# couchbase/blance

Measured on AMD Instinct MI355X. Metric: partition-state assignments/sec at 1M partitions x 4,096 nodes, higher is better.
Workload: dtype f64

## Files before the change

### __graft_entry__.py

```python
import os
import subprocess
import sys

ROOT = os.path.dirname(os.path.abspath(__file__))
if ROOT not in sys.path:
    sys.path.insert(0, ROOT)

CSRC = os.path.join(ROOT, "blance_amd", "csrc")
HIP_TUS = ["blance_hip.hip", "tu_seq.hip", "tu_tree.hip", "tu_queue.hip", "tu_chain.hip", "tu_batch.hip"]
HIP_LIB = os.path.join(ROOT, "blance_amd", "lib", "libblance_hip.so")
HIP_OBJ = os.path.join(ROOT, "blance_amd", "lib", "obj")
HIPCC_FLAGS = ["--offload-arch=gfx950", "-O3", "-std=c++17", "-ffp-contract=off", "-fPIC"]


def _stale(target, deps):
    return (not os.path.exists(target)) or any(os.path.getmtime(d) > os.path.getmtime(target) for d in deps)


def depfile_entries(path):
    try:
        with open(path) as f:
            text = f.read()
    except OSError:
        return None
# ... 159 lines not shown
    if not force and stamp is not None and os.path.exists(lib) and _read(lib + ".stamp") == stamp:
        return lib
    os.makedirs(os.path.dirname(lib), exist_ok=True)
    hipcc = os.environ.get("HIPCC", "/opt/rocm/bin/hipcc")
    for old in (lib + ".d", lib + ".deps", lib + ".stamp"):
        if os.path.exists(old):
            os.remove(old)
    r = subprocess.run([hipcc] + HIPCC_FLAGS + ["-shared", "-MD", "-MF", lib + ".d", "-o", lib, src],
                       stderr=subprocess.PIPE, text=True)
    if r.returncode != 0:
        err = "\n".join(l for l in (r.stderr or "").splitlines() if "error" in l.lower())
        raise RuntimeError("hipcc failed on %s\n%s" % (src, err[-4000:]))
    deps = depfile_entries(lib + ".d") or []
    rels = sorted(set(os.path.relpath(os.path.realpath(d), os.path.realpath(ROOT)) for d in deps if not d.startswith(("/opt/", "/usr/"))))
    with open(lib + ".deps", "w") as f:
        f.write("\n".join(rels) + "\n")
    with open(lib + ".stamp", "w") as f:
        f.write(_small_stamp(lib))
    return lib


def build_stay_rank_cases(force=False):
    return _build_small_cases(RANKS_SRC, RANKS_LIB, force)


PERIOD_SRC = os.path.join(CASES_DIR, "period_cases.hip")
PERIOD_LIB = os.path.join(CASES_DIR, "_build", "libblance_period_cases.so")


def build_period_cases(force=False):
    return _build_small_cases(PERIOD_SRC, PERIOD_LIB, force)


def build_host():
    host = os.path.join(ROOT, "blance_amd", "csrc", "host")
    srcs = [os.path.join(host, "blance_host_cli.cpp"), os.path.join(host, "blance_api.cpp"), os.path.join(host, "call_arena.cpp")]
    out = os.path.join(ROOT, "blance_amd", "lib", "blance_host_cli")
    if _stale(out, srcs + [os.path.join(host, "blance_api.hpp"), os.path.join(host, "call_arena.hpp"),
                           os.path.join(ROOT, "include", "blance_hip.h")]):
        subprocess.check_call(["g++", "-std=c++17", "-O2", "-pthread", "-DBLANCE_CALL_ARENA", "-o", out] + srcs + ["-ldl"])
    build_wire()
    build_move_index()
    return out


def build_move_index():
    host = os.path.join(ROOT, "blance_amd", "csrc", "host")
    src, hdr = os.path.join(host, "move_index_sim.cpp"), os.path.join(host, "move_index.hpp")
    out = os.path.join(ROOT, "blance_amd", "lib", "move_index_sim")
    if _stale(out, [src, hdr]):
        subprocess.check_call(["g++", "-std=c++17", "-O2", "-o", out, src])
    return out


def build_wire():
    src = os.path.join(ROOT, "blance_amd", "csrc", "host", "blance_wire.cpp")
    out = os.path.join(ROOT, "blance_amd", "lib", "libblance_wire.so")
    if _stale(out, [src, os.path.join(ROOT, "include", "blance_wire.h"),
                    os.path.join(ROOT, "blance_amd", "csrc", "host", "json_escape.hpp")]):
        subprocess.check_call(["g++", "-std=c++17", "-O2", "-fPIC", "-shared", "-I", os.path.join(ROOT, "include"),
                               "-o", out, src])
    return out


def build():
    with_cases = os.path.exists(CASES_SRC) and all(os.path.exists(os.path.join(CASES_DIR, inc)) for inc in CASES_INCS)
    cases = start_kernel_cases() if with_cases else None
    try:
        build_hip()
    except BaseException:
        if cases is not None:
            cases.kill()
        raise
    if with_cases:
        build_kernel_cases(cases)
    if os.path.exists(RANKS_SRC):
        build_stay_rank_cases()
    if os.path.exists(PERIOD_SRC):
        build_period_cases()
    build_host()
    from oracle import loader, naive_loader
    loader.build()
    naive_loader.build()
    from blance_amd import hip
    lib = hip.load_library()
    assert lib.blance_abi_version() == 6
    import blance_amd


def smoke():
    from blance_amd import hip, synth
    from oracle import loader
    fp = synth.config_flat(3, P=2048, N=256)
    pl = hip.Planner(device_id=0)
    got = pl.plan(fp)
    want = loader.plan(fp)
    assert got.digest() == want.digest(), "HIP result differs from the oracle"
    assert got.iterations == want.iterations
    fp2 = synth.config_flat(2, P=4096, N=64)
    assert pl.plan(fp2).digest() == loader.plan(fp2).digest()
    fp3 = synth.config5_initial(3000, 128)
    r3 = pl.plan(fp3)
    assert r3.digest() == loader.plan(fp3).digest(), "config-5-shaped plan differs from the oracle"
    fp4 = synth.config5_rebalance(fp3, r3, 3000, 128)
    assert pl.plan(fp4).digest() == loader.plan(fp4).digest(), "config-5-shaped rebalance differs from the oracle"
    pl.close()
    print("smoke ok: iterations=%d device_ms=%.3f" % (got.iterations, got.struct.device_ms))


if __name__ == "__main__":
    build()
    if len(sys.argv) > 1 and sys.argv[1] == "smoke":
# ... 2 lines not shown
```

### blance_amd/csrc/blance_hip.hip

```cpp
#include "dev_prelude.h"

#include <algorithm>
#include <atomic>
#include <chrono>
#include <map>
#include <mutex>
#include <new>
#include <thread>
#include <type_traits>
#include <string>
#include <vector>

#include "k_sweep.h"
#include "k_flat.h"
#include "k_period.h"
#include "k_plan_moves.h"
#include "k_plan_wire.h"
#include "host/json_escape.hpp"
#ifdef BLANCE_SIMT_EMU
#include "tu_seq.hip"
#include "tu_tree.hip"
#include "tu_queue.hip"
#include "tu_chain.hip"
#include "tu_batch.hip"
#endif


using namespace blance;

static thread_local std::string g_last_error;

static int fail(int code, const char* fmt, const char* a = "", long b = 0) {
    char buf[512];
    snprintf(buf, sizeof buf, fmt, a, b);
    g_last_error = buf;
    return code;
}

#define HIPTRY(expr)                                                                  \
    do {                                                                              \
        hipError_t e_ = (expr);                                                       \
        if (e_ != hipSuccess)                                                         \
            return fail(BLANCE_ERR_DEVICE, "%s failed: line %ld", hipGetErrorString(e_), __LINE__); \
    } while (0)

struct DevBuf {
    void* p = nullptr;
    size_t cap = 0;
// ... 168 lines not shown
};

constexpr int kChainHandoffMin = 8192;

enum PassKind { kPassKernel = 0, kPassFlatBulk = 1, kPassBlank = 2, kPassStayTop = 3 };

struct blance_ctx : CtxHandles {
    int device = 0;
    int engine = BLANCE_ENGINE_AUTO;
    int force_threads = 0;
    std::mutex mu;
    bool uploaded = false;
    bool planned = false;
    blance_comm comm{0, 1, nullptr, nullptr, nullptr};
    void* rccl_comm = nullptr;
    DevBuf scan_sums;
    DevBuf scan_part;
    DevBuf topkey, top_counts, top_off, top_order;
    DevBuf side_sums;
    bool side_pending = false;
    int top_group_state = -1;
    int64_t top_group_epoch = -1, group_epoch = 0;
    std::vector<int64_t> last_stays;
    int chain_handoff = kChainHandoffMin;
    DevBuf handoff;
    bool no_stay_top = false;
    bool force_stay_top = false;
    bool periodic = true;
    int periodic_cut = 0;
    bool period_known = true;
    uint32_t assign_kinds = 0;
    bool cycle_order_stands = false;
    bool leaves_distinct = false;
    DevBuf cnt_base, xbuf, gath;
    std::vector<int32_t> h_reg_off;
    int chain_group_state = -1;
    bool chain_group_static = false;
    bool tops_moved = true;
    uint32_t top_gate = 0;
    bool flags_clean = false;
    bool rowcount_clean = false;
    bool top_prio_strict = false;
    bool uniform_first = false, uniform_all = false;
    bool trace = false;
    int dump_sweep = -1;
    DevBuf dl_off, dl_nodes;
    HostStage stage;
    void* rb_buf = nullptr;
    size_t rb_used = 0;
    struct RbItem { void* dst; size_t off, bytes; };
    std::vector<RbItem> rb_items;
    DevBuf vres, vseen;
    DevBuf mv[11];
    bool wire_names = false;
    int wire_stage = kWireStageDefault;
    DevBuf wire[10];
    int64_t comm_calls = 0, comm_bytes = 0;
    size_t comm_events_used = 0;
    double comm_ms = 0.0;
    int64_t n_syncs = 0;
    bool assign_empty = false, counts_start_zero = false;
    int chain_waves = 0;
    int speculate = 1;
    bool fused_tail = true;

    blance_problem h{};
    std::vector<int32_t> state_priority, state_constraints, rule_off;
    int L = 1, np_later = 0, n_alive = 0, any_removed = 0;
    int chain_min_parts = 2048;
    int any_node_weight = 0;
    bool no_fast_keys = false;
    bool no_seq_spec = false;
    bool no_tree = false;
    bool tree_dense = false;
    bool tree_always = false;
    bool tree_long = false;
    bool no_planes = false;
    bool no_queue = false;
    bool queue_general = false;
    bool queue_no_asm = false;
    bool queue_force_dense = false;
    bool queue_exact_rebuild = false;
    bool queue_bits_self = false;
    bool shard_one_rank = false;
    DevBuf ntn_bits;
    bool bits_stale = false;
    bool pass_ntn_ready = false;
    int64_t queue_launches = 0, queue_stops = 0, queue_moved = 0, queue_exact = 0, queue_rebuilds = 0, queue_dense = 0;
    struct RuleRegions {
        bool ok = false;
        int n_regions = 0, max_size = 0;
        DevBuf node_region, reg_lo, reg_hi, leaf_cls, cls_size;
        DevBuf wg_region, wg_chunk;
        int n_stay_wgs = 0, n_leaves = 0;
        int cls_run = 0;
    };
    std::vector<RuleRegions> rule_regions;
    DevBuf leaf_node, regid, chain_order, bucket_counts, reg_off, cnt_save, crec;
    DevBuf chain_inv;
    DevBuf period, cnt_p1;
    DevBuf fl_iota, fl_zero, fl_one, fl_reglo, fl_reghi;
    DevBuf n_ev, chain_oi, ev_key, ev_oi, ev_leaf, ev_w, ev_perm, ev_off, ev_counts;
    bool flat_chain_ok = false;
    DevBuf f_tot, f_g, f_top_g, f_top_n, f_row_count, f_m, f_moff, f_keys_a, f_keys_b, f_vals_a, f_vals_b, f_hist, f_comp;
    int64_t out_capacity = 0;
    DevBuf batch_in, batch_sc, batch_out;

    DevBuf node_removed, node_added, node_weight, node_has_weight, alive, zeros_nx, node_leaf_pos;
    DevBuf alive_ids, alive_rank;
    DevBuf part_order, part_weight, part_has_weight, part_in_prev, part_never_equal;
    DevBuf a_off, a_nodes, a_kind, p_off, p_nodes, p_kind;
    DevBuf load_state, load_node, load_weight, load_first;
    DevBuf rule_inc, rule_exc, vparent, vlo, vhi, anchors;
    DevBuf state_stick, state_has_stick;
    DevBuf live, live_len, live_kind, prv, prv_len, prv_kind, in_prev, never_equal;
    DevBuf cnt, ntn, cat, order, chunk_counts, rec, out, warn_part, warn_state, scalars;
    DevBuf cnt_next;
    bool tail_counted = false;
    PlanStats stats;
    ~blance_ctx();
    std::vector<PassKind> pass_kind;
};

static void comm_release(blance_ctx* c);
template <class F>
static int guarded(F f) {
    try {
        return f();
// ... 150 lines not shown
    if (!out) return fail(BLANCE_ERR_BAD_ARG, "null out");
    *out = nullptr;
    int n_dev = 0;
    if (hipGetDeviceCount(&n_dev) != hipSuccess || n_dev <= 0)
        return fail(BLANCE_ERR_NO_DEVICE, "no HIP device visible");
    int dev = opt ? opt->device_id : 0;
    if (dev < 0 || dev >= n_dev) return fail(BLANCE_ERR_BAD_ARG, "device_id out of range");
    HIPTRY(hipSetDevice(dev));
    blance_ctx* c = new blance_ctx();
    c->device = dev;
    c->engine = opt ? opt->engine : BLANCE_ENGINE_AUTO;
    c->force_threads = opt ? opt->reserved[0] : 0;
    if (opt && opt->reserved[1] > 0) c->chain_min_parts = opt->reserved[1];
    c->no_seq_spec = opt && (opt->reserved[2] & 1);
    c->no_tree = opt && (opt->reserved[2] & 2);
    c->tree_dense = opt && (opt->reserved[2] & 4);
    c->tree_always = opt && (opt->reserved[2] & 8);
    c->tree_long = opt && (opt->reserved[2] & 16);
    c->no_planes = opt && (opt->reserved[2] & 32);
    c->no_queue = opt && (opt->reserved[2] & 512);
    c->queue_general = opt && (opt->reserved[2] & 1024);
    c->queue_force_dense = opt && (opt->reserved[2] & 2048);
    c->queue_no_asm = opt && (opt->reserved[2] & 4096);
    c->queue_exact_rebuild = opt && (opt->reserved[2] & 8192);
    c->shard_one_rank = opt && (opt->reserved[2] & 16384);
    c->queue_bits_self = opt && (opt->reserved[2] & 32768);
    c->no_stay_top = opt && (opt->reserved[2] & 64);
    c->force_stay_top = opt && (opt->reserved[2] & 128);
    c->periodic = !(opt && (opt->reserved[2] & 256));
    if (const char* pe = getenv("BLANCE_PERIODIC")) c->periodic = atoi(pe) != 0;
    if (const char* pc = getenv("BLANCE_PERIODIC_CUT")) c->periodic_cut = atoi(pc);
    c->period_known = !(opt && (opt->reserved[2] & 65536));
    if (const char* pk = getenv("BLANCE_PERIOD_KNOWN")) c->period_known = atoi(pk) != 0;
    c->trace = getenv("BLANCE_TRACE") != nullptr;
    if (const char* cw = getenv("BLANCE_CHAIN_WAVES")) c->chain_waves = atoi(cw);
    if (const char* ho = getenv("BLANCE_CHAIN_HANDOFF")) c->chain_handoff = atoi(ho) > 0 ? atoi(ho) : 0;
    if (const char* sp = getenv("BLANCE_SPECULATE")) c->speculate = !strcmp(sp, "fail") ? 2 : atoi(sp) != 0;
    if (const char* ft = getenv("BLANCE_FUSED_TAIL")) c->fused_tail = atoi(ft) != 0;
    if (const char* ds = getenv("BLANCE_DUMP_SWEEP")) c->dump_sweep = atoi(ds);
    if (const char* ws = getenv("BLANCE_WIRE_STAGE")) {
        const int v = atoi(ws);
        c->wire_stage = v < kWireStageMin ? kWireStageMin : v > kWireStageMax ? kWireStageMax : v;
    }
    if (hipStreamCreate(&c->stream) != hipSuccess || hipEventCreate(&c->ev0) != hipSuccess ||
        hipEventCreate(&c->ev1) != hipSuccess ||
        hipEventCreate(&c->side_go) != hipSuccess || hipEventCreate(&c->side_done) != hipSuccess) {
        delete c;
        return fail(BLANCE_ERR_DEVICE, "stream/event creation failed");
    }
    *out = c;
    g_live_contexts++;
    return BLANCE_OK;
}

blance_ctx::~blance_ctx() {
    (void)hipSetDevice(device);
    if (stream) (void)hipStreamSynchronize(stream);
    if (side) (void)hipStreamSynchronize(side);
    comm_release(this);
    if (rb_buf) pin_free(rb_buf);
}

extern "C" void blance_ctx_destroy(blance_ctx* c) {
    if (!c) return;
    delete c;
    if (--g_live_contexts == 0) pin_trim();
// ... 360 lines not shown
                    if (sz != cls_run || sz < 1 || sz > 64 || (sz & (sz - 1)) || (cl[i].first - rlo[g]) % sz) cls_run = 0;
                    for (int lp = cl[i].first; lp < cl[i].second && cls_run > 0; lp++) if (leaf_node[lp] < 0) cls_run = 0;
                }
                for (size_t i = 0; i < cl.size() && ok; i++) cls_size[rlo[g] + i] = cl[i].second - cl[i].first;
                for (int lp = rlo[g]; lp < rhi[g] && ok; lp++) {
                    int a = leaf_node[lp];
                    if (a < 0) continue;
                    size_t j = std::upper_bound(cl.begin(), cl.end(), std::make_pair(lp, INT_MAX)) - cl.begin();
                    if (j > 0 && lp < cl[j - 1].second) {
                        if (t[a].blo != cl[j - 1].first || t[a].bhi != cl[j - 1].second) ok = false;
                        leaf_cls[lp] = (int)j - 1;
                    }
                }
            }
            rr.ok = ok;
            rr.n_regions = ok ? (int)rlo.size() : 0;
            rr.max_size = max_size;
            rr.n_leaves = n_leaves;
            rr.cls_run = ok && cls_run > 0 ? cls_run : 0;
            std::vector<int32_t> wg_region, wg_chunk;
            if (ok)
                for (size_t g = 0; g < rlo.size(); g++)
                    for (int ch = 0; ch * 64 < rhi[g] - rlo[g]; ch++) { wg_region.push_back((int32_t)g); wg_chunk.push_back(ch); }
            rr.n_stay_wgs = (int)wg_region.size();
            if (ok) {
                if (put(up, rr.wg_region, wg_region.data(), wg_region.size())) return BLANCE_ERR_DEVICE;
                if (put(up, rr.wg_chunk, wg_chunk.data(), wg_chunk.size())) return BLANCE_ERR_DEVICE;
                if (put(up, rr.node_region, node_region.data(), node_region.size())) return BLANCE_ERR_DEVICE;
                if (put(up, rr.reg_lo, rlo.data(), rlo.size())) return BLANCE_ERR_DEVICE;
                if (put(up, rr.reg_hi, rhi.data(), rhi.size())) return BLANCE_ERR_DEVICE;
                if (put(up, rr.leaf_cls, leaf_cls.data(), leaf_cls.size())) return BLANCE_ERR_DEVICE;
                if (put(up, rr.cls_size, cls_size.data(), cls_size.size())) return BLANCE_ERR_DEVICE;
            }
            if ((st = up.flush())) return st;
        }
        if ((st = up.flush())) return st;
    }
    const int RW = kRecHead + M * (1 + L);
    int kmax = 1;
    for (int m = 0; m < M; m++) if (pb->state_constraints[m] > kmax) kmax = pb->state_constraints[m];
    RESERVE(live, sizeof(int32_t) * (size_t)(PM * L + 1));
    RESERVE(live_len, sizeof(int32_t) * (size_t)(PM + 1));
    RESERVE(live_kind, (size_t)PM + 1);
    RESERVE(prv, sizeof(int32_t) * (size_t)(PM * L + 1));
    RESERVE(prv_len, sizeof(int32_t) * (size_t)(PM + 1));
    RESERVE(prv_kind, (size_t)PM + 1);
    RESERVE(in_prev, (size_t)P + 1);
    RESERVE(never_equal, (size_t)P + 1);
    RESERVE(cnt, sizeof(int32_t) * (size_t)(M + 1) * (NX + 1));
    RESERVE(cnt_next, sizeof(int32_t) * (size_t)(M + 1) * (NX + 1));
    RESERVE(ntn, sizeof(int32_t) * (size_t)(NX + 1) * (N > 0 ? N : 1));
    RESERVE(cat, (size_t)P + 1);
    RESERVE(order, sizeof(int32_t) * ((size_t)P + 1));
    RESERVE(chunk_counts, sizeof(int32_t) * 3 * (size_t)(cdiv(P, kPartChunk) + 1));
    RESERVE(rec, sizeof(int32_t) * ((size_t)P * RW + 64));
    RESERVE(out, sizeof(int32_t) * ((size_t)P * (1 + kmax) + 1));
    RESERVE(warn_part, sizeof(int32_t) * (size_t)(PM + 1));
    RESERVE(warn_state, sizeof(int32_t) * (size_t)(PM + 1));
    RESERVE(scalars, sizeof(int32_t) * kScalWords);
    RESERVE(ntn_bits, sizeof(uint32_t) * (queue_bits_words(NX) + 4));
    {
        int maxB = 1;
        for (auto& rr : c->rule_regions) if (rr.ok && rr.n_regions > maxB) maxB = rr.n_regions;
        RESERVE(regid, sizeof(int32_t) * ((size_t)P + 1));
        RESERVE(chain_order, sizeof(int32_t) * ((size_t)P + 1));
        RESERVE(chain_inv, sizeof(int32_t) * ((size_t)P + 1));
// ... 730 lines not shown
    d.live = d.prv; d.live_len = d.prv_len; d.live_kind = d.prv_kind;
    return d;
}

static DevProblem dev_problem(blance_ctx* c) {
    const blance_problem& h = c->h;
    DevProblem d;
    d.N = h.n_nodes; d.NX = h.n_nodes_ext; d.M = h.n_states; d.L = c->L; d.P = h.n_parts;
    d.weights_nil = h.partition_weights_nil;
    d.node_removed = c->zeros_nx.as<uint8_t>();
    d.node_added = c->zeros_nx.as<uint8_t>();
    d.part_weight = c->part_weight.as<int32_t>();
    d.part_has_weight = c->part_has_weight.as<uint8_t>();
    d.live = c->live.as<int32_t>(); d.live_len = c->live_len.as<int32_t>(); d.live_kind = c->live_kind.as<uint8_t>();
    d.prv = c->prv.as<int32_t>(); d.prv_len = c->prv_len.as<int32_t>(); d.prv_kind = c->prv_kind.as<uint8_t>();
    d.in_prev = c->in_prev.as<uint8_t>(); d.never_equal = c->never_equal.as<uint8_t>();
    return d;
}

constexpr int kXHead = 16, kXPoison = kChainFlags;
struct SweepTail {
    bool set = false, scatter = false;
    int m = 0, OW = 0;
    const int32_t* order = nullptr;
    const int32_t* inv = nullptr;
    Gate gate = kNoGate;
};
struct ChainPassArgs {
    int m, k, NP, higher_mask, r0, it;
    const int32_t* order;
    bool same_tops;
    SweepTail* tail;
    bool known_cycle = false;
};

static void comm_poison(blance_ctx* c) {
    const blance_problem& h = c->h;
    const size_t n = kXHead + (size_t)(h.n_states + 1) * h.n_nodes_ext;
    if (c->xbuf.reserve(sizeof(int32_t) * (n + 1))) return;
    if (hipMemsetAsync(c->xbuf.p, 0, sizeof(int32_t) * n, c->stream) != hipSuccess) return;
    const int32_t one = 1;
    if (hipMemcpyAsync(c->xbuf.as<int32_t>() + kXPoison, &one, sizeof one, hipMemcpyHostToDevice, c->stream) != hipSuccess) return;
    if (stream_sync(c) != hipSuccess) return;
    (void)comm_allreduce(c, c->xbuf.as<int32_t>(), (int64_t)n);
    (void)stream_sync(c);
}

struct Progress {
    int64_t steps = 0, batched = 0;
    int n_pass = 0;
    int passes_this_sweep = 0;
};
struct PlanRun {
    DevProblem d;
    int64_t launches = 0;
    Progress at;
    int32_t hs[kScalReadback] = {0};
    int m_last = -1;
    bool fuse = false;
    bool top_spec_plan = true;
    bool handoff_plan = true;
    int iterations = 0, converged = 0;
};

enum class Pending { kNone, kStayTop, kBlank, kChain };
struct ChainRun {
    bool allow_spec = true, defer = false, no_stay = false, no_lean = false, skip = false;
    bool no_handoff = false;
    bool handoff = false;
    bool redo_handoff = false;
    bool redo = false;
    Pending pending = Pending::kNone;
    bool spec = false;
    Gate gate = kNoGate;
    bool done = false;
    bool a_done = false;
};

struct ChainPass {
    blance_ctx* const c;
    PlanRun& pr;
    const ChainPassArgs& a;
    ChainRun& run;
    const blance_problem& h;
    const DevProblem& d;
    blance_ctx::RuleRegions& rr;
    const int m, OW, P, B, nbc, G, rank;
    const bool sharded;
    const size_t cnt_words;
    const hipStream_t sm;
    int32_t* const flags;
    Gate top_gate = kNoGate;
    bool regroup = false, spec = false, defer = false, gather_out = false;
    int32_t cfl[kChainFlags] = {0};
    int32_t n_events = 0;
    bool stay_fits = false, try_stay = false, group_stands = false, group_ahead = false;
    bool handoff = false;
    ChainParams cq;

    ChainPass(blance_ctx* c_, PlanRun& pr_, const ChainPassArgs& a_, ChainRun& run_)
        : c(c_), pr(pr_), a(a_), run(run_), h(c_->h), d(pr_.d), rr(c_->rule_regions[a_.r0]), m(a_.m), OW(1 + a_.k), P(c_->h.n_parts), B(rr.n_regions),
          nbc(cdiv(c_->h.n_parts, kPartChunk)), G(c_->comm.n_ranks), rank(c_->comm.rank), sharded(pass_sharded(c_, rr.n_regions)),
          cnt_words((size_t)(c_->h.n_states + 1) * c_->h.n_nodes_ext), sm(c_->stream),
          flags(c_->scalars.as<int32_t>() + kScalFlags) {}

    int slice_lo(int r) const { return (int)((int64_t)B * r / G); }
    Gate gate_on(uint32_t words) const {
        return Gate{flags, words | (1u << kFlagForced) | (spec ? (1u << kFlagOrphans) | (1u << kFlagEvents) : 0u) | c->top_gate};
    }
    bool refuted(const int32_t* f) const { return spec && (f[kFlagOrphans] || f[kFlagEvents] || c->speculate == 2); }
    void uncount_orphans() {
        BLANCE_LAUNCH_NOSYNC(k_chain_orphans, cdiv(P, 256), 256, 0, sm, d, m, h.top_state, a.order,
                             rr.node_region.as<int32_t>(), c->cnt.as<int32_t>());
    }
    int restore_counters() {
        HIPTRY(hipMemcpyAsync(c->cnt.p, c->cnt_save.p, sizeof(int32_t) * cnt_words, hipMemcpyDeviceToDevice, sm));
        return 0;
    }
    int open_timing() { HIPTRY(hipEventRecord(c->pass_events[2 * pr.at.n_pass], sm)); return 0; }
    int close_timing(PassKind kind) {
        HIPTRY(hipEventRecord(c->pass_events[2 * pr.at.n_pass + 1], sm));
        c->pass_kind.resize(pr.at.n_pass + 1);
        c->pass_kind[pr.at.n_pass] = kind;
        pr.at.n_pass++;
        return 0;
    }

    int classify_and_group();
    int events();
    int gather_records();
    int group_by_top(hipStream_t st, DevBuf& sums);
    void fill_chain_params();
    int start_counters();
    void fill_stay_params(StayParams& sq);
    int stay_attempt(bool* stayed);
    int stay_behind_handoff();
    int trace_handoff();
    int longest_chain() const {
        int mx = 0;
        if (c->h_reg_off.size() == (size_t)B + 1)
            for (int r = 0; r < B; r++) mx = std::max(mx, (int)(c->h_reg_off[r + 1] - c->h_reg_off[r]));
        return mx;
    }
    int blank_walk(bool* lean);
    int periodic_walk(bool* walked);
    int collective_a(int32_t* fl);
    int collective_b();
    int commit();
    int run_once();
};

int ChainPass::classify_and_group() {
    if (!c->flags_clean) HIPTRY(hipMemsetAsync(flags, 0, sizeof(int32_t) * kChainFlags, sm));
    c->flags_clean = false;
    top_gate = Gate{flags, c->top_gate};
    regroup = !(a.same_tops && c->chain_group_state == m && c->chain_group_static && a.order == c->part_order.as<int32_t>() &&
                c->h_reg_off.size() == (size_t)B + 1);
    spec = run.allow_spec && !regroup && !sharded && c->speculate > 0;
    if (!spec) {
        const LaunchShape cs = shape_chain_classify(P);
        BLANCE_LAUNCH_NOSYNC(k_chain_classify, cs.grid, cs.block, cs.lds, sm, d, m, h.top_state,
                             a.order, rr.node_region.as<int32_t>(), c->regid.as<int32_t>(),
                             c->n_ev.as<int32_t>(), flags, top_gate);
    } else {
        if (c->trace) fprintf(stderr, "[blance] chain pass state %d: no k_chain_classify, k_gather_chain raises its flag words\n", m);
    }
    if (regroup) {
        const int ge = group_by_key(c, sm, c->scan_sums, P, c->regid.as<int32_t>(), a.order, B, c->bucket_counts.as<int32_t>(),
                                    c->reg_off.as<int32_t>(), c->chain_order.as<int32_t>(), c->chain_oi.as<int32_t>());
        if (ge) return ge;
        BLANCE_LAUNCH_NOSYNC(k_invert, cdiv(P, 256), 256, 0, sm, P, c->chain_order.as<int32_t>(), c->chain_inv.as<int32_t>());
        pr.launches++;
        c->chain_group_state = m;
        c->group_epoch++;
        c->chain_group_static = a.order == c->part_order.as<int32_t>();
    } else if (c->trace) fprintf(stderr, "[blance] chain pass state %d: the grouping by region of the last sweep stands\n", m);
    defer = run.defer && !sharded && c->speculate > 0;
    if (c->top_gate && (regroup || !spec || !defer))
        return fail(BLANCE_ERR_DEVICE, "a chain pass behind the top-state pass's verdict would read back");
    run.spec = spec;
    run.pending = Pending::kNone;
    run.redo = false;
    if (!spec) {
        HIPTRY(read_back(c, cfl, flags, sizeof cfl));
        if (regroup) {
            c->h_reg_off.resize((size_t)B + 1);
            HIPTRY(read_back(c, c->h_reg_off.data(), c->reg_off.p, sizeof(int32_t) * ((size_t)B + 1)));
        }
        HIPTRY(stream_sync(c));
    }
    return 0;
}

int ChainPass::events() {
    if (!cfl[kFlagNotLocal] && cfl[kFlagEvents]) {
        SCANTRY(P + 1, c->n_ev.as<int32_t>());
        HIPTRY(read_back(c, &n_events, c->n_ev.as<int32_t>() + P, sizeof n_events));
        HIPTRY(stream_sync(c));
    }
    if (c->trace)
        fprintf(stderr, spec ? "[blance] chain pass state %d: classification assumed clean (checked with the pass's flags)\n" :
                               "[blance] chain pass state %d: %d events, not-local %d, orphans %d\n", m, n_events, cfl[kFlagNotLocal], cfl[kFlagOrphans]);
    {
        FillCopyJob fj;
        fj.zero(c->ev_off.p, (int64_t)B + 1);
        fj.zero(flags + kFlagStayMoved, 1);
        fj.zero(flags + kFlagHandedOff, 1);
        fj.copy(c->cnt_save.p, c->cnt.p, (int64_t)cnt_words);
        if (run_fill_copy(c, fj)) return BLANCE_ERR_DEVICE;
    }
    if (!cfl[kFlagNotLocal] && n_events > 0) {
        BLANCE_LAUNCH_NOSYNC(k_chain_ev_fill, cdiv(P, 256), 256, 0, sm, d, m, h.top_state, a.order,
                             rr.node_region.as<int32_t>(), rr.reg_lo.as<int32_t>(), c->node_leaf_pos.as<int32_t>(),
                             c->regid.as<int32_t>(), c->n_ev.as<int32_t>(), c->ev_key.as<int32_t>(),
                             c->ev_oi.as<int32_t>(), c->ev_leaf.as<int32_t>(), c->ev_w.as<int32_t>());
        const int ge = group_by_key(c, sm, c->scan_sums, n_events, c->ev_key.as<int32_t>(), nullptr, B, c->ev_counts.as<int32_t>(),
                                    c->ev_off.as<int32_t>(), c->ev_perm.as<int32_t>(), nullptr);
        if (ge) return ge;
        pr.launches += 5;
    }
    return 0;
}

int ChainPass::group_by_top(hipStream_t st, DevBuf& sums) {
    const int ge = group_by_key(c, st, sums, P, c->topkey.as<int32_t>(), nullptr, rr.n_leaves, c->top_counts.as<int32_t>(),
                                c->top_off.as<int32_t>(), c->top_order.as<int32_t>(), nullptr);
    if (ge) return ge;
    c->top_group_state = m;
    c->top_group_epoch = c->group_epoch;
    pr.launches += 5;
    return 0;
}

int ChainPass::gather_records() {
    const bool fits_but_np = !sharded && !c->no_stay_top && !cfl[kFlagNotLocal] && !cfl[kFlagOrphans] && !cfl[kFlagEvents] &&
                             rr.max_size <= kStayMaxLeaves && rr.n_stay_wgs > 0;
    stay_fits = fits_but_np && a.NP > 0;
    try_stay = stay_fits && !run.no_stay && (c->force_stay_top || c->last_stays[m] * 100 >= (int64_t)P * 99);
    const bool handoff_plan_ok = c->chain_handoff > 0 && pr.handoff_plan && c->speculate > 0 && !run.no_handoff && run.allow_spec &&
                                 longest_chain() - 64 * 4 >= c->chain_handoff;
    handoff = stay_fits && !try_stay && handoff_plan_ok && chain_rows_in_lds(cq, rr.max_size);
    const bool handoff_next = fits_but_np && a.NP == 0 && c->np_later > 0 && handoff_plan_ok && a.it + 1 < h.max_iterations;
    group_stands = c->top_group_state == m && c->top_group_epoch == c->group_epoch;
    const bool for_next = stay_fits && !try_stay && c->speculate > 0 && a.it + 1 < h.max_iterations;
    group_ahead = (for_next || handoff || handoff_next) && !group_stands && (c->side || g_live_contexts.load() <= 2);
    if (group_ahead && !c->side && hipStreamCreate(&c->side) != hipSuccess) { c->side = nullptr; group_ahead = false; (void)hipGetLastError(); }
    const bool group_here = (handoff || handoff_next) && !group_stands && !group_ahead;
    if (try_stay || group_ahead || handoff || group_here) {
        RESERVE(topkey, sizeof(int32_t) * ((size_t)P + 1));
        RESERVE(top_order, sizeof(int32_t) * ((size_t)P + 1));
        RESERVE(top_off, sizeof(int32_t) * ((size_t)rr.n_leaves + 2));
        RESERVE(top_counts, sizeof(int32_t) * ((size_t)rr.n_leaves * nbc + 1));
        if (c->side_pending) {
            HIPTRY(hipStreamWaitEvent(sm, c->side_done, 0));
            c->side_pending = false;
        }
    }
    const bool group_now = (try_stay && !group_stands) || group_ahead || group_here;
    const LaunchShape gs = shape_gather_chain(P);
    BLANCE_LAUNCH(k_gather_chain, gs.grid, gs.block, gs.lds, sm, d, m, h.top_state, a.higher_mask,
                         c->chain_order.as<int32_t>(), c->chain_oi.as<int32_t>(), c->state_stick.as<int32_t>(),
                         c->state_has_stick.as<uint8_t>(), c->node_leaf_pos.as<int32_t>(),
                         rr.node_region.as<int32_t>(), rr.reg_lo.as<int32_t>(), rr.leaf_cls.as<int32_t>(),
                         rr.cls_size.as<int32_t>(), 0, spec ? 1 : 0,
                         c->crec.as<int32_t>(), flags, group_now ? c->topkey.as<int32_t>() : (int32_t*)nullptr, top_gate);
    if (group_ahead) {
        HIPTRY(hipEventRecord(c->side_go, sm));
        HIPTRY(hipStreamWaitEvent(c->side, c->side_go, 0));
        const int ge = group_by_top(c->side, c->side_sums);
        if (ge) return ge;
        HIPTRY(hipEventRecord(c->side_done, c->side));
        c->side_pending = true;
        if (c->trace) fprintf(stderr, "[blance] chain pass state %d: the steps grouped by top priority node for the next sweep, on the second stream\n", m);
    } else if (group_here) {
        const int ge = group_by_top(sm, c->scan_sums);
        if (ge) return ge;
        if (c->trace) fprintf(stderr, "[blance] chain pass state %d: the steps grouped by top priority node for the hand-off\n", m);
    }
    return 0;
}

void ChainPass::fill_chain_params() {
    fill_pass_common(c, cq, m, a.k, a.NP);
    fill_region_tables(c, rr, cq);
    cq.L = c->L;
    cq.n_regions = B;
    cq.waves = c->chain_waves ? c->chain_waves : (a.it == 0 ? 4 : 0);
    cq.cls_run = rr.cls_run;
    cq.region_base = sharded ? slice_lo(rank) : 0;
    cq.n_launch = sharded ? slice_lo(rank + 1) - cq.region_base : B;
    cq.reg_off = c->reg_off.as<int32_t>();
    cq.ntn = c->ntn.as<int32_t>();
    cq.crec = c->crec.as<int32_t>(); cq.out = c->out.as<int32_t>();
    cq.flags = flags;
    cq.gate = c->top_gate;
    cq.ev_off = c->ev_off.as<int32_t>(); cq.ev_perm = c->ev_perm.as<int32_t>();
    cq.ev_oi = c->ev_oi.as<int32_t>(); cq.ev_leaf = c->ev_leaf.as<int32_t>(); cq.ev_w = c->ev_w.as<int32_t>();
    cq.cnt_out = cq.cnt;
}

int ChainPass::start_counters() {
    if (cfl[kFlagOrphans]) uncount_orphans();
    gather_out = sharded && (c->comm.allgather_i32 || !c->comm.allreduce_sum_i32);
    if (sharded) {
        RESERVE(cnt_base, sizeof(int32_t) * (cnt_words + 1));
        RESERVE(xbuf, sizeof(int32_t) * (kXHead + cnt_words + 1));
        HIPTRY(hipMemcpyAsync(c->cnt_base.p, c->cnt.p, sizeof(int32_t) * cnt_words, hipMemcpyDeviceToDevice, sm));
        if (!gather_out) HIPTRY(hipMemsetAsync(c->out.p, 0, sizeof(int32_t) * (size_t)P * OW, sm));
    }
    return 0;
// ... 24 lines not shown
    if (!launch_stay_by_top(sm, sq, rr.n_stay_wgs, rr.max_size)) return fail(BLANCE_ERR_UNSUPPORTED, "k_stay_by_top shape behind a hand-off");
    pr.launches += 1;
    return close_timing(kPassStayTop);
}

int ChainPass::trace_handoff() {
    std::vector<int32_t> at((size_t)B), ro((size_t)B + 1);
    HIPTRY(hipMemcpyAsync(at.data(), c->handoff.p, sizeof(int32_t) * at.size(), hipMemcpyDeviceToHost, sm));
    HIPTRY(hipMemcpyAsync(ro.data(), c->reg_off.p, sizeof(int32_t) * ro.size(), hipMemcpyDeviceToHost, sm));
    HIPTRY(stream_sync(c));
    std::string line;
    int n = 0;
    if (B > 0 && at[0] < 0) {
        fprintf(stderr, "[blance] chain pass state %d: hand-off (%d steps or more): the launch returned at its gate, no region walked\n", m, c->chain_handoff);
        return 0;
    }
    for (int r = 0; r < B; r++) {
        char buf[96];
        if (at[r] >= ro[r] && at[r] < ro[r + 1]) {
            snprintf(buf, sizeof buf, " region %d at step %d of %d;", r, at[r] - ro[r], ro[r + 1] - ro[r]);
            n++;
        } else {
            snprintf(buf, sizeof buf, " region %d walked to its end (%d);", r, ro[r + 1] - ro[r]);
        }
        line += buf;
    }
    fprintf(stderr, "[blance] chain pass state %d: hand-off (%d steps or more) in %d of %d regions:%s\n", m, c->chain_handoff, n, B, line.c_str());
    return 0;
}

int ChainPass::stay_attempt(bool* stayed) {
    *stayed = false;
    if (!group_stands) {
        const int ge = group_by_top(sm, c->scan_sums);
        if (ge) return ge;
    } else if (c->trace) fprintf(stderr, "[blance] chain pass state %d: the steps' grouping by top priority node stands\n", m);
    StayParams sq;
    fill_stay_params(sq);
    if (!launch_stay_by_top(sm, sq, rr.n_stay_wgs, rr.max_size)) return 0;
    pr.launches += 1;
    if (defer) {
        *stayed = true;
        run.pending = Pending::kStayTop;
        run.gate = gate_on((1u << kFlagNotLocal) | (1u << kFlagStayMoved));
        if (c->trace) fprintf(stderr, "[blance] chain pass state %d: stays per top priority node, the verdict is read with the sweep's\n", m);
        return 0;
    }
    int32_t sf[kChainFlags] = {0}, moved = 0;
    HIPTRY(read_back(c, sf, flags, sizeof sf));
    HIPTRY(read_back(c, &moved, flags + kFlagStayMoved, sizeof moved));
    HIPTRY(stream_sync(c));
    if (refuted(sf)) {
        run.redo = true;
        return 0;
    }
    *stayed = !sf[kFlagNotLocal] && !moved;
    if (c->trace) fprintf(stderr, "[blance] chain pass state %d: stays verified per top priority node: %s\n", m, *stayed ? "all of them" : "no");
    return 0;
}

int ChainPass::periodic_walk(bool* walked) {
    const int N = h.n_nodes, NX = h.n_nodes_ext;
    *walked = false;
    int max_len = 0;
    for (int r = 0; r < B; r++) max_len = std::max(max_len, (int)(c->h_reg_off[r + 1] - c->h_reg_off[r]));
    if (max_len < kPeriodMinRounds * 2) return 0;
    RESERVE(period, sizeof(int32_t) * ((size_t)kPWords * B + 1));
// ... 424 lines not shown
    return 0;
}

static int run_state_pass(blance_ctx* c, PlanRun& pr, Sweep& sw, int m) {
    const blance_problem& h = c->h;
    const int M = h.n_states, P = h.n_parts;
    StatePass sp;
    sp.m = m;
    sp.k = c->state_constraints[m];
    if (sw.restore_counters) {
        HIPTRY(hipMemcpyAsync(c->cnt.p, c->cnt_save.p, sizeof(int32_t) * (size_t)(M + 1) * h.n_nodes_ext, hipMemcpyDeviceToDevice, c->stream));
        sw.restore_counters = false;
    }
    const int oe = pass_order(c, pr, sw, m, &sp.order);
    if (oe) return oe;
    pr.at.passes_this_sweep++;
    c->pass_ntn_ready = false;
    sp.higher_mask = 0;
    for (int t = 0; t < M; t++)
        if (c->state_priority[t] < c->state_priority[m]) sp.higher_mask |= 1 << t;
    sp.r0 = c->rule_off[m]; sp.r1 = c->rule_off[m + 1];
    while (c->pass_events.size() < 2 * (size_t)(pr.at.n_pass + 3)) {
        hipEvent_t ev;
        HIPTRY(hipEventCreate(&ev));
        c->pass_events.push_back(ev);
    }
    bool done = false;
    if (c->engine != BLANCE_ENGINE_SEQUENTIAL && !h.hierarchy_rules_nil && sp.r1 - sp.r0 == 1 &&
        c->rule_regions[sp.r0].ok && P >= c->chain_min_parts && sp.k <= 4 && !(sw.retrying && sw.retry.skip)) {
        ChainPassArgs ca{m, sp.k, sw.NP, sp.higher_mask, sp.r0, sw.it, sp.order,
                         !sw.first && !c->tops_moved && m != h.top_state && c->top_prio_strict,
                         pr.fuse && m == pr.m_last ? &sw.tail : nullptr};
        const uint32_t kinds_m = (c->assign_kinds >> m) & 0x10001u;
        ca.known_cycle = c->period_known && sw.first && !sw.retrying && !sw.known_broken && pr.at.passes_this_sweep == 2 &&
                         sw.known_passes == 1 && sw.known_cycle && sw.known_state == h.top_state && sw.known_k == 1 &&
                         m != h.top_state && sw.NP == 0 && c->assign_empty && h.partition_weights_nil && c->cycle_order_stands &&
                         c->leaves_distinct && kinds_m != 0x10001u;
        ChainRun run;
        if (sw.retrying) run = sw.retry;
        run.defer = !sw.retrying && m == pr.m_last;
        sw.known_broken = true;
        const int e = run_chain_pass(c, pr, ca, run);
        if (e) {
            const bool sharded = pass_sharded(c, c->rule_regions[sp.r0].n_regions);
            if (sharded && !run.a_done) comm_poison(c);
            if (sharded) comm_abort(c);
            return e;
        }
        if (run.pending != Pending::kNone) sw.pend = run;
        done = run.done;
    }
    if (!done) {
        const int e = run_pass_in_order(c, pr, sw, sp);
        if (e) return e;
    }
    pr.launches += 7;
    pr.at.steps += P;
    return 0;
}

static int close_sweep(blance_ctx* c, PlanRun& pr, Sweep& sw) {
    const blance_problem& h = c->h;
    const int P = h.n_parts;
    if (P <= 0) return 0;
    hipStream_t sm = c->stream;
    int32_t* scal = c->scalars.as<int32_t>();
    const DevProblem& d = pr.d;
    SweepTail& tail = sw.tail;
    const Gate cg = sw.pend.pending != Pending::kNone ? sw.pend.gate : c->top_gate ? Gate{scal + kScalFlags, c->top_gate} : kNoGate;
    if (tail.set && tail.scatter && (!tail.inv || tail.gate.flags != cg.flags || tail.gate.mask != cg.mask)) {
// ... 1185 lines not shown
```

### blance_amd/hip.py

```python
import ctypes as C
import os

from . import abi

_HERE = os.path.dirname(os.path.abspath(__file__))
LIB_PATH = os.path.join(_HERE, "lib", "libblance_hip.so")

EXPORTS = ["blance_abi_version", "blance_last_error", "blance_result_capacity", "blance_validate",
           "blance_ctx_create", "blance_ctx_destroy", "blance_plan", "blance_upload",
           "blance_plan_resident", "blance_download", "blance_calc_moves", "blance_plan_stats_get",
           "blance_comm_unique_id", "blance_comm_init_rccl", "blance_comm_set", "blance_comm_stats",
           "blance_is_emulated", "blance_host_alloc", "blance_host_free", "blance_comm_time_ms", "blance_host_trim",
           "blance_plan_moves_capacity", "blance_plan_moves_get", "blance_plan_wire_names", "blance_plan_wire_get"]

_libs = {}


class BlanceError(RuntimeError):
    def __init__(self, status, text):
        RuntimeError.__init__(self, "blance status %d: %s" % (status, text))
        self.status = status


def load_library(path=None):
# ... 122 lines not shown
        except Exception:
            pass


class HostArena:

    def __init__(self, lib_path=None):
        self.lib = load_library(lib_path)
        self.n_blocks = 0

    def empty(self, n, dtype):
        import numpy as np
        dt = np.dtype(dtype)
        nbytes = max(int(n), 1) * dt.itemsize
        block = _PinnedBlock(self.lib, nbytes)
        buf = (C.c_char * nbytes).from_address(block.p)
        buf._block = block
        self.n_blocks += 1
        return np.frombuffer(buf, dtype=dt, count=int(n))

    def copy_of(self, arr):
        a = self.empty(arr.size, arr.dtype)
        a[...] = arr.reshape(-1)
        return a

    def close(self):
        """Kept for callers of the earlier interface: the blocks are owned by the arrays, nothing to release here."""


class Planner:

    def __init__(self, device_id=0, engine=abi.ENGINE_AUTO, lib_path=None, force_threads=0,
                 chain_min_parts=0, seq_speculation=True, tree="auto", planes=True, stay_top="auto", periodic=True, queue=True,
                 shard_one_rank=False, period_known=True):
        self.lib = load_library(lib_path)
        opt = abi.Options()
        opt.engine = engine
        opt.device_id = device_id
        opt.reserved[0] = force_threads
        opt.reserved[1] = chain_min_parts
        qbits = {True: 0, "on": 0, False: 512, "off": 512, "general": 1024, "dense": 1024 | 2048, "lean-cpp": 4096,
                 "exact-rebuild": 8192, "bits-self": 32768}[queue]
        opt.reserved[2] = qbits | (16384 if shard_one_rank else 0) | (0 if period_known else 65536) | (0 if periodic else 256) | {"auto": 0, "off": 64, "force": 128}[stay_top] | (0 if planes else 32) | (0 if seq_speculation else 1) | {"auto": 0, "off": 2, "dense": 4 | 8, "on": 8, "long": 8 | 16,
                                                          "dense-long": 4 | 8 | 16}[tree]
        h = C.c_void_p()
        self._check(self.lib.blance_ctx_create(C.byref(opt), C.byref(h)))
        self._h = h

    def _check(self, st):
        if st != abi.OK:
            raise BlanceError(st, (self.lib.blance_last_error() or b"").decode())

    def close(self):
        if getattr(self, "_h", None):
            self.lib.blance_ctx_destroy(self._h)
            self._h = None

    def __del__(self):
        try:
            self.close()
        except Exception:
            pass

    def comm_init_rccl(self, dist):
        rank, world = dist.get_rank(), dist.get_world_size()
        buf = C.create_string_buffer(128)
        if rank == 0:
            self._check(self.lib.blance_comm_unique_id(buf))
        box = [buf.raw]
        dist.broadcast_object_list(box, src=0)
        ident = C.create_string_buffer(box[0], 128)
        self._check(self.lib.blance_comm_init_rccl(self._h, world, rank, ident))
        return world

    def comm_init_rccl_one_rank(self):
        buf = C.create_string_buffer(128)
# ... 288 lines not shown
```

Measured before the change: 3.560 billion.

## Group chain-pass steps by region and top node from round-robin tables, skip sorts

When the first sweep's assignment is a known round robin over alive nodes, the host precomputes per-node tables (region, rank within region, leaf, count) and region/leaf offsets at upload. The chain pass then scatters each partition directly to its grouped slot with one kernel instead of a key sort, and builds the top-priority grouping with a direct-index kernel instead of group_by_top. This also drops the readback of region offsets. A flag check falls back and drops the grouping if the tables do not match the actual tops, at the cost of extra host table building and new code paths.

```diff
diff --git a/__graft_entry__.py b/__graft_entry__.py
--- a/__graft_entry__.py
+++ b/__graft_entry__.py
@@ -215,6 +215,14 @@
     return _build_small_cases(PERIOD_SRC, PERIOD_LIB, force)
 
 
+CYCLE_SRC = os.path.join(CASES_DIR, "cycle_cases.hip")
+CYCLE_LIB = os.path.join(CASES_DIR, "_build", "libblance_cycle_cases.so")
+
+
+def build_cycle_cases(force=False):
+    return _build_small_cases(CYCLE_SRC, CYCLE_LIB, force)
+
+
 def build_host():
     host = os.path.join(ROOT, "blance_amd", "csrc", "host")
     srcs = [os.path.join(host, "blance_host_cli.cpp"), os.path.join(host, "blance_api.cpp"), os.path.join(host, "call_arena.cpp")]
@@ -261,6 +269,8 @@
         build_stay_rank_cases()
     if os.path.exists(PERIOD_SRC):
         build_period_cases()
+    if os.path.exists(CYCLE_SRC):
+        build_cycle_cases()
     build_host()
     from oracle import loader, naive_loader
     loader.build()
diff --git a/blance_amd/csrc/blance_hip.hip b/blance_amd/csrc/blance_hip.hip
--- a/blance_amd/csrc/blance_hip.hip
+++ b/blance_amd/csrc/blance_hip.hip
@@ -14,6 +14,7 @@
 #include "k_sweep.h"
 #include "k_flat.h"
 #include "k_period.h"
+#include "k_cycle.h"
 #include "k_plan_moves.h"
 #include "k_plan_wire.h"
 #include "host/json_escape.hpp"
@@ -248,6 +249,8 @@
     uint32_t assign_kinds = 0;
     bool cycle_order_stands = false;
     bool leaves_distinct = false;
+    int cycle_group = 1;
+    int64_t cycle_group_epoch = -1;
     DevBuf cnt_base, xbuf, gath;
     std::vector<int32_t> h_reg_off;
     int chain_group_state = -1;
@@ -310,6 +313,9 @@
         DevBuf wg_region, wg_chunk;
         int n_stay_wgs = 0, n_leaves = 0;
         int cls_run = 0;
+        bool cyc_ok = false;
+        DevBuf cyc, cyc_reg_off, cyc_top_off;
+        std::vector<int32_t> h_cyc_reg_off;
     };
     std::vector<RuleRegions> rule_regions;
     DevBuf leaf_node, regid, chain_order, bucket_counts, reg_off, cnt_save, crec;
@@ -526,6 +532,8 @@
     if (const char* pc = getenv("BLANCE_PERIODIC_CUT")) c->periodic_cut = atoi(pc);
     c->period_known = !(opt && (opt->reserved[2] & 65536));
     if (const char* pk = getenv("BLANCE_PERIOD_KNOWN")) c->period_known = atoi(pk) != 0;
+    c->cycle_group = opt && (opt->reserved[2] & 131072) ? 0 : 1;
+    if (const char* cg = getenv("BLANCE_CYCLE_GROUP")) c->cycle_group = !strcmp(cg, "refute") ? 2 : atoi(cg) != 0;
     c->trace = getenv("BLANCE_TRACE") != nullptr;
     if (const char* cw = getenv("BLANCE_CHAIN_WAVES")) c->chain_waves = atoi(cw);
     if (const char* ho = getenv("BLANCE_CHAIN_HANDOFF")) c->chain_handoff = atoi(ho) > 0 ? atoi(ho) : 0;
@@ -952,6 +960,34 @@
                 if (put(up, rr.leaf_cls, leaf_cls.data(), leaf_cls.size())) return BLANCE_ERR_DEVICE;
                 if (put(up, rr.cls_size, cls_size.data(), cls_size.size())) return BLANCE_ERR_DEVICE;
             }
+            rr.cyc_ok = false;
+            std::vector<int32_t> cyc, cyc_top_off;
+            if (ok && c->leaves_distinct && c->n_alive >= 1) {
+                const int A = c->n_alive, B = (int)rlo.size(), full = P / A, part = P % A;
+                bool all_in = true;
+                for (int a = 0; a < A && all_in; a++) all_in = node_region[alive_ids[a]] >= 0;
+                if (all_in) {
+                    std::vector<int32_t> count((size_t)B, 0), last((size_t)B, 0), leaf_steps((size_t)n_leaves, 0);
+                    cyc.assign((size_t)A * kCycWords, 0);
+                    for (int a = 0; a < A; a++) {
+                        const int n = alive_ids[a], g = node_region[n];
+                        cyc[(size_t)a * kCycWords + kCycRegion] = g;
+                        cyc[(size_t)a * kCycWords + kCycRank] = count[g]++;
+                        cyc[(size_t)a * kCycWords + kCycLeaf] = pb->node_leaf_pos[n];
+                        if (a < part) last[g]++;
+                        leaf_steps[pb->node_leaf_pos[n]] = full + (a < part ? 1 : 0);
+                    }
+                    for (int a = 0; a < A; a++) cyc[(size_t)a * kCycWords + kCycCount] = count[cyc[(size_t)a * kCycWords + kCycRegion]];
+                    rr.h_cyc_reg_off.assign((size_t)B + 1, 0);
+                    for (int g = 0; g < B; g++) rr.h_cyc_reg_off[g + 1] = rr.h_cyc_reg_off[g] + full * count[g] + last[g];
+                    cyc_top_off.assign((size_t)n_leaves + 1, 0);
+                    for (int lp = 0; lp < n_leaves; lp++) cyc_top_off[lp + 1] = cyc_top_off[lp] + leaf_steps[lp];
+                    if (put(up, rr.cyc, cyc.data(), cyc.size())) return BLANCE_ERR_DEVICE;
+                    if (put(up, rr.cyc_reg_off, rr.h_cyc_reg_off.data(), rr.h_cyc_reg_off.size())) return BLANCE_ERR_DEVICE;
+                    if (put(up, rr.cyc_top_off, cyc_top_off.data(), cyc_top_off.size())) return BLANCE_ERR_DEVICE;
+                    rr.cyc_ok = true;
+                }
+            }
             if ((st = up.flush())) return st;
         }
         if ((st = up.flush())) return st;
@@ -1748,6 +1784,7 @@
     bool same_tops;
     SweepTail* tail;
     bool known_cycle = false;
+    bool round_robin = false;
 };
 
 static void comm_poison(blance_ctx* c) {
@@ -1808,6 +1845,7 @@
     int32_t* const flags;
     Gate top_gate = kNoGate;
     bool regroup = false, spec = false, defer = false, gather_out = false;
+    bool cycle = false;
     int32_t cfl[kChainFlags] = {0};
     int32_t n_events = 0;
     bool stay_fits = false, try_stay = false, group_stands = false, group_ahead = false;
@@ -1846,6 +1884,8 @@
     int events();
     int gather_records();
     int group_by_top(hipStream_t st, DevBuf& sums);
+    bool top_from_tables() const;
+    int top_by_tables();
     void fill_chain_params();
     int start_counters();
     void fill_stay_params(StayParams& sq);
@@ -1873,7 +1913,21 @@
     regroup = !(a.same_tops && c->chain_group_state == m && c->chain_group_static && a.order == c->part_order.as<int32_t>() &&
                 c->h_reg_off.size() == (size_t)B + 1);
     spec = run.allow_spec && !regroup && !sharded && c->speculate > 0;
-    if (!spec) {
+    cycle = a.round_robin && regroup && !sharded && rr.cyc_ok && c->cycle_group > 0 && a.order != nullptr;
+    if (cycle) {
+        const LaunchShape cs = shape_chain_classify(P);
+        BLANCE_LAUNCH_NOSYNC(k_cycle_group, cs.grid, cs.block, cs.lds, sm, d, m, h.top_state, a.order, rr.node_region.as<int32_t>(),
+                             c->n_alive, B, c->alive_ids.as<int32_t>(), rr.cyc.as<int32_t>(), rr.cyc_reg_off.as<int32_t>(),
+                             c->cycle_group == 2 ? 1 : 0, c->regid.as<int32_t>(), c->n_ev.as<int32_t>(),
+                             c->chain_order.as<int32_t>(), c->chain_oi.as<int32_t>(), c->chain_inv.as<int32_t>(),
+                             c->reg_off.as<int32_t>(), flags, top_gate);
+        pr.launches++;
+        c->chain_group_state = m;
+        c->group_epoch++;
+        c->chain_group_static = a.order == c->part_order.as<int32_t>();
+        c->cycle_group_epoch = c->group_epoch;
+        if (c->trace) fprintf(stderr, "[blance] chain pass state %d: the steps grouped by region from the round robin's tables, no sort\n", m);
+    } else if (!spec) {
         const LaunchShape cs = shape_chain_classify(P);
         BLANCE_LAUNCH_NOSYNC(k_chain_classify, cs.grid, cs.block, cs.lds, sm, d, m, h.top_state,
                              a.order, rr.node_region.as<int32_t>(), c->regid.as<int32_t>(),
@@ -1881,7 +1935,7 @@
     } else {
         if (c->trace) fprintf(stderr, "[blance] chain pass state %d: no k_chain_classify, k_gather_chain raises its flag words\n", m);
     }
-    if (regroup) {
+    if (regroup && !cycle) {
         const int ge = group_by_key(c, sm, c->scan_sums, P, c->regid.as<int32_t>(), a.order, B, c->bucket_counts.as<int32_t>(),
                                     c->reg_off.as<int32_t>(), c->chain_order.as<int32_t>(), c->chain_oi.as<int32_t>());
         if (ge) return ge;
@@ -1890,7 +1944,7 @@
         c->chain_group_state = m;
         c->group_epoch++;
         c->chain_group_static = a.order == c->part_order.as<int32_t>();
-    } else if (c->trace) fprintf(stderr, "[blance] chain pass state %d: the grouping by region of the last sweep stands\n", m);
+    } else if (!regroup && c->trace) fprintf(stderr, "[blance] chain pass state %d: the grouping by region of the last sweep stands\n", m);
     defer = run.defer && !sharded && c->speculate > 0;
     if (c->top_gate && (regroup || !spec || !defer))
         return fail(BLANCE_ERR_DEVICE, "a chain pass behind the top-state pass's verdict would read back");
@@ -1899,11 +1953,19 @@
     run.redo = false;
     if (!spec) {
         HIPTRY(read_back(c, cfl, flags, sizeof cfl));
-        if (regroup) {
+        if (cycle) {
+            c->h_reg_off = rr.h_cyc_reg_off;
+        } else if (regroup) {
             c->h_reg_off.resize((size_t)B + 1);
             HIPTRY(read_back(c, c->h_reg_off.data(), c->reg_off.p, sizeof(int32_t) * ((size_t)B + 1)));
         }
         HIPTRY(stream_sync(c));
+    }
+    if (cycle && cfl[kFlagNotLocal]) {
+        c->chain_group_state = -1;
+        c->top_group_state = -1;
+        c->cycle_group_epoch = -1;
+        if (c->trace) fprintf(stderr, "[blance] chain pass state %d: the round robin's tables do not describe this pass, the grouping is dropped\n", m);
     }
     return 0;
 }
@@ -1945,6 +2007,22 @@
     c->top_group_state = m;
     c->top_group_epoch = c->group_epoch;
     pr.launches += 5;
+    return 0;
+}
+
+bool ChainPass::top_from_tables() const {
+    return c->cycle_group > 0 && rr.cyc_ok && !sharded && c->chain_group_state == m && c->cycle_group_epoch == c->group_epoch &&
+           !cfl[kFlagNotLocal];
+}
+int ChainPass::top_by_tables() {
+    const int A = c->n_alive, wpa = std::max(1, cdiv(cdiv(P, A), 64));
+    BLANCE_LAUNCH_NOSYNC(k_cycle_top, cdiv((int64_t)A * wpa, 4), 256, 0, sm, P, A, wpa, rr.n_leaves, rr.cyc.as<int32_t>(),
+                         rr.cyc_reg_off.as<int32_t>(), rr.cyc_top_off.as<int32_t>(), c->top_off.as<int32_t>(),
+                         c->top_order.as<int32_t>(), top_gate);
+    c->top_group_state = m;
+    c->top_group_epoch = c->group_epoch;
+    pr.launches += 5;
+    if (c->trace) fprintf(stderr, "[blance] chain pass state %d: the steps grouped by top priority node from the round robin's tables, no sort\n", m);
     return 0;
 }
 
@@ -1960,9 +2038,12 @@
     group_stands = c->top_group_state == m && c->top_group_epoch == c->group_epoch;
     const bool for_next = stay_fits && !try_stay && c->speculate > 0 && a.it + 1 < h.max_iterations;
     group_ahead = (for_next || handoff || handoff_next) && !group_stands && (c->side || g_live_contexts.load() <= 2);
+    const bool by_tables = top_from_tables();
+    const bool list_by_tables = by_tables && (group_ahead || ((handoff || handoff_next) && !group_stands));
+    if (by_tables) group_ahead = false;
     if (group_ahead && !c->side && hipStreamCreate(&c->side) != hipSuccess) { c->side = nullptr; group_ahead = false; (void)hipGetLastError(); }
-    const bool group_here = (handoff || handoff_next) && !group_stands && !group_ahead;
-    if (try_stay || group_ahead || handoff || group_here) {
+    const bool group_here = (handoff || handoff_next) && !group_stands && !group_ahead && !by_tables;
+    if (try_stay || group_ahead || handoff || group_here || list_by_tables) {
         RESERVE(topkey, sizeof(int32_t) * ((size_t)P + 1));
         RESERVE(top_order, sizeof(int32_t) * ((size_t)P + 1));
         RESERVE(top_off, sizeof(int32_t) * ((size_t)rr.n_leaves + 2));
@@ -1972,7 +2053,7 @@
             c->side_pending = false;
         }
     }
-    const bool group_now = (try_stay && !group_stands) || group_ahead || group_here;
+    const bool group_now = (try_stay && !group_stands && !by_tables) || group_ahead || group_here;
     const LaunchShape gs = shape_gather_chain(P);
     BLANCE_LAUNCH(k_gather_chain, gs.grid, gs.block, gs.lds, sm, d, m, h.top_state, a.higher_mask,
                          c->chain_order.as<int32_t>(), c->chain_oi.as<int32_t>(), c->state_stick.as<int32_t>(),
@@ -1992,6 +2073,9 @@
         const int ge = group_by_top(sm, c->scan_sums);
         if (ge) return ge;
         if (c->trace) fprintf(stderr, "[blance] chain pass state %d: the steps grouped by top priority node for the hand-off\n", m);
+    } else if (list_by_tables) {
+        const int ge = top_by_tables();
+        if (ge) return ge;
     }
     return 0;
 }
@@ -2082,7 +2166,7 @@
 int ChainPass::stay_attempt(bool* stayed) {
     *stayed = false;
     if (!group_stands) {
-        const int ge = group_by_top(sm, c->scan_sums);
+        const int ge = top_from_tables() ? top_by_tables() : group_by_top(sm, c->scan_sums);
         if (ge) return ge;
     } else if (c->trace) fprintf(stderr, "[blance] chain pass state %d: the steps' grouping by top priority node stands\n", m);
     StayParams sq;
@@ -2573,10 +2657,11 @@
                          !sw.first && !c->tops_moved && m != h.top_state && c->top_prio_strict,
                          pr.fuse && m == pr.m_last ? &sw.tail : nullptr};
         const uint32_t kinds_m = (c->assign_kinds >> m) & 0x10001u;
-        ca.known_cycle = c->period_known && sw.first && !sw.retrying && !sw.known_broken && pr.at.passes_this_sweep == 2 &&
+        ca.round_robin = sw.first && !sw.retrying && !sw.known_broken && pr.at.passes_this_sweep == 2 &&
                          sw.known_passes == 1 && sw.known_cycle && sw.known_state == h.top_state && sw.known_k == 1 &&
                          m != h.top_state && sw.NP == 0 && c->assign_empty && h.partition_weights_nil && c->cycle_order_stands &&
                          c->leaves_distinct && kinds_m != 0x10001u;
+        ca.known_cycle = c->period_known && ca.round_robin;
         ChainRun run;
         if (sw.retrying) run = sw.retry;
         run.defer = !sw.retrying && m == pr.m_last;
diff --git a/blance_amd/csrc/k_cycle.h b/blance_amd/csrc/k_cycle.h
--- /dev/null
+++ b/blance_amd/csrc/k_cycle.h
@@ -0,0 +1,60 @@
+#pragma once
+
+namespace blance {
+
+constexpr int kCycWords = 4;
+constexpr int kCycRegion = 0, kCycRank = 1, kCycLeaf = 2, kCycCount = 3;
+
+__global__ void k_cycle_group(DevProblem d, int m, int top_state, const int32_t* order, const int32_t* node_region, int A,
+                              int B, const int32_t* alive_ids, const int32_t* cyc ,
+                              const int32_t* reg_off_tab, int refute, int32_t* regid, int32_t* n_ev, int32_t* chain_order,
+                              int32_t* chain_oi, int32_t* chain_inv, int32_t* reg_off_out, int32_t* flags, Gate gate) {
+    if (gate_closed(gate)) return;
+    const int oi = blockIdx.x * blockDim.x + threadIdx.x;
+    for (int j = oi; j <= B; j += gridDim.x * blockDim.x) reg_off_out[j] = reg_off_tab[j];
+    if (oi > d.P) return;
+    if (oi == d.P) { n_ev[oi] = 0; return; }
+    const int p = order[oi];
+    const int idxT = p * d.M + top_state;
+    const int top = (d.live_kind[idxT] != kListAbsent && d.live_len[idxT] > 0) ? d.live[(size_t)idxT * d.L] : -1;
+    int rg = top >= 0 ? node_region[top] : -1;
+    int ne = 0;
+    if (rg >= 0) {
+        const int idx = p * d.M + m;
+        if (d.live_kind[idx] != kListAbsent)
+            for (int i = 0; i < d.live_len[idx]; i++) {
+                const int r2 = node_region[d.live[(size_t)idx * d.L + i]];
+                if (r2 == rg) continue;
+                if (r2 >= 0) ne++; else flags[kFlagOrphans] = 1;
+                flags[kFlagEvents] = 1;
+            }
+    }
+    if (rg < 0) { flags[kFlagNotLocal] = 1; rg = 0; }
+    regid[oi] = rg;
+    n_ev[oi] = ne;
+    const int s = oi / A, a = oi - s * A;
+    const int expect = alive_ids[refute && oi == 0 ? (oi + 1) % A : a];
+    if (top != expect) flags[kFlagNotLocal] = 1;
+    const int32_t* t = cyc + (size_t)a * kCycWords;
+    const int i = reg_off_tab[t[kCycRegion]] + s * t[kCycCount] + t[kCycRank];
+    chain_order[i] = p;
+    chain_oi[i] = oi;
+    chain_inv[p] = i;
+}
+
+__global__ void k_cycle_top(int P, int A, int waves_per_a, int n_leaves, const int32_t* cyc, const int32_t* reg_off_tab,
+                            const int32_t* top_off_tab, int32_t* top_off_out, int32_t* top_order, Gate gate) {
+    if (gate_closed(gate)) return;
+    const int tid = blockIdx.x * blockDim.x + threadIdx.x;
+    for (int j = tid; j <= n_leaves; j += gridDim.x * blockDim.x) top_off_out[j] = top_off_tab[j];
+    const int w = tid >> 6, lane = tid & 63;
+    const int a = w / waves_per_a;
+    if (a >= A) return;
+    const int s = (w - a * waves_per_a) * 64 + lane;
+    const int count = P / A + (a < P % A ? 1 : 0);
+    if (s >= count) return;
+    const int32_t* t = cyc + (size_t)a * kCycWords;
+    top_order[top_off_tab[t[kCycLeaf]] + s] = reg_off_tab[t[kCycRegion]] + s * t[kCycCount] + t[kCycRank];
+}
+
+}
diff --git a/blance_amd/hip.py b/blance_amd/hip.py
--- a/blance_amd/hip.py
+++ b/blance_amd/hip.py
@@ -178,7 +178,7 @@
 
     def __init__(self, device_id=0, engine=abi.ENGINE_AUTO, lib_path=None, force_threads=0,
                  chain_min_parts=0, seq_speculation=True, tree="auto", planes=True, stay_top="auto", periodic=True, queue=True,
-                 shard_one_rank=False, period_known=True):
+                 shard_one_rank=False, period_known=True, cycle_group=True):
         self.lib = load_library(lib_path)
         opt = abi.Options()
         opt.engine = engine
@@ -187,7 +187,7 @@
         opt.reserved[1] = chain_min_parts
         qbits = {True: 0, "on": 0, False: 512, "off": 512, "general": 1024, "dense": 1024 | 2048, "lean-cpp": 4096,
                  "exact-rebuild": 8192, "bits-self": 32768}[queue]
-        opt.reserved[2] = qbits | (16384 if shard_one_rank else 0) | (0 if period_known else 65536) | (0 if periodic else 256) | {"auto": 0, "off": 64, "force": 128}[stay_top] | (0 if planes else 32) | (0 if seq_speculation else 1) | {"auto": 0, "off": 2, "dense": 4 | 8, "on": 8, "long": 8 | 16,
+        opt.reserved[2] = qbits | (16384 if shard_one_rank else 0) | (0 if period_known else 65536) | (0 if cycle_group else 131072) | (0 if periodic else 256) | {"auto": 0, "off": 64, "force": 128}[stay_top] | (0 if planes else 32) | (0 if seq_speculation else 1) | {"auto": 0, "off": 2, "dense": 4 | 8, "on": 8, "long": 8 | 16,
                                                           "dense-long": 4 | 8 | 16}[tree]
         h = C.c_void_p()
         self._check(self.lib.blance_ctx_create(C.byref(opt), C.byref(h)))
```

New measurement: 4.286 billion, median of 6. 20.4% higher.
